# automl/TransformersCanDoBayesianInference

Hardware: AMD Instinct MI355X
Metric: synthetic datasets/sec (GP prior, bptt=2000) (higher is better)
Workload: dtype fp16; 1 GPU; priors.fast_gp, bptt=2000, num_features=18, emsize=512, nhead=4, nhid=1024, nlayers=6, 1000 bars (BASELINE.json configs[1]); per_gpu_batch=64, global_batch=64, aggregate_k_gradients=1, aggregate_streams=0, aggregate_stacked=False, seq_len=2000, parallelism=dp1, micro_batch_streams=2, eval_pos=weighted sampler(2000)

## Files before the change

transformerscandobayesianinference_amd/csrc/gemm_tn.hip:

```cpp
#include <type_traits>
#include "pfn_device.h"
#include "pfn_kernels.h"

namespace pfn {

PFN_DEV int xcd_remap(int bid, int nwg) {
  const int q = nwg >> 3, r = nwg & 7, xcd = bid & 7;
  return (xcd < r ? xcd * (q + 1) : r * (q + 1) + (xcd - r) * q) + (bid >> 3);
}
typedef __attribute__((address_space(1))) const void gvoid_t;
typedef __attribute__((address_space(3))) void lvoid_t;

constexpr int TN_BMK = 32;

template <typename T>
__global__ __launch_bounds__(256, 2) void gemm_tn_kernel(GemmTN g) {
  constexpr int RB = 128 * sizeof(T);
  constexpr int TILE = TN_BMK * RB;
  extern __shared__ __attribute__((aligned(16))) char smem_raw[];
  LdsPtr smem = lds_cast(smem_raw);
  auto tileA = [&](int buf) { return smem + buf * 2 * TILE; };
  auto tileB = [&](int buf) { return smem + buf * 2 * TILE + TILE; };

  const int p0 = blockIdx.y * 128, q0 = blockIdx.x * 128;
  const int colsA = min(128, g.P - p0), colsB = min(128, g.Q - q0);
  const long mbeg = (long)blockIdx.z * g.m_chunk;
  const long mend = min((long)g.M, mbeg + g.m_chunk);
  if (mbeg >= mend) return;
  const T* A = reinterpret_cast<const T*>(g.A) + mbeg * g.lda + p0;
  const T* B = reinterpret_cast<const T*>(g.B) + mbeg * g.ldb + q0;

  const int wave = threadIdx.x >> 6, lane = threadIdx.x & 63;
  const int wp = wave >> 1, wq = wave & 1;

  f32x16 acc[2][2];
#pragma unroll
  for (int i = 0; i < 2; ++i)
#pragma unroll
    for (int j = 0; j < 2; ++j)
#pragma unroll
      for (int r = 0; r < 16; ++r) acc[i][j][r] = 0.f;

  TileStage<T, TN_BMK, RB, 256> sa, sb;
  const int rows_total = (int)(mend - mbeg);
  const int nt = (rows_total + TN_BMK - 1) / TN_BMK;
  const bool do_colsum = g.colsum != nullptr && blockIdx.x == 0;
  constexpr int EPC = 16 / sizeof(T);
  float csum[EPC];
#pragma unroll
  for (int e = 0; e < EPC; ++e) csum[e] = 0.f;
  auto add_colsum = [&]() {
    if (!do_colsum) return;
#pragma unroll
    for (int i = 0; i < sa.PER; ++i) {
      if constexpr (sizeof(T) == 2) {
        const X8<T> v = __builtin_bit_cast(X8<T>, sa.regs[i]);
#pragma unroll
        for (int e = 0; e < 8; ++e) csum[e] += (float)v[e];
      } else {
        const f32x4 v = __builtin_bit_cast(f32x4, sa.regs[i]);
#pragma unroll
        for (int e = 0; e < 4; ++e) csum[e] += v[e];
      }
    }
  };
  sa.issue(A, g.lda, rows_total, colsA);
  sb.issue(B, g.ldb, rows_total, colsB);
  add_colsum();
  sa.template commit<true>(tileA(0));
  sb.template commit<true>(tileB(0));
  __syncthreads();
  for (int t = 0; t < nt; ++t) {
    const int cur = t & 1;
    if (t + 1 < nt) {
      const long r1 = (long)(t + 1) * TN_BMK;
      sa.issue(A + r1 * g.lda, g.lda, rows_total - (int)r1, colsA);
      sb.issue(B + r1 * g.ldb, g.ldb, rows_total - (int)r1, colsB);
      add_colsum();
    }
    const lds_char* ta = tileA(cur);
    const lds_char* tb = tileB(cur);
#pragma unroll
    for (int ks = 0; ks < TN_BMK; ks += 16) {
      Frag<T> fa[2], fb[2];
#pragma unroll
      for (int i = 0; i < 2; ++i) fa[i] = load_frag_tr<T, RB, 1>(ta, ks, wp * 64 + i * 32);
#pragma unroll
      for (int j = 0; j < 2; ++j) fb[j] = load_frag_tr<T, RB, 1>(tb, ks, wq * 64 + j * 32);
#pragma unroll
      for (int i = 0; i < 2; ++i)
#pragma unroll
        for (int j = 0; j < 2; ++j) acc[i][j] = mma32(fa[i], fb[j], acc[i][j]);
    }
    if (t + 1 < nt) {
      sa.template commit<true>(tileA(cur ^ 1));
      sb.template commit<true>(tileB(cur ^ 1));
    }
    __syncthreads();
  }

  const float osc = loss_scale_down(g.scale_amax);
  if (do_colsum) {
    constexpr int NCH = RB / 16;
    float* red = reinterpret_cast<float*>(smem_raw);
#pragma unroll
    for (int e = 0; e < EPC; ++e) red[threadIdx.x * EPC + e] = csum[e];
    __syncthreads();
    if (threadIdx.x < NCH) {
#pragma unroll
      for (int e = 0; e < EPC; ++e) {
        float t = 0.f;
        for (int j = 0; j < 256 / NCH; ++j) t += red[(j * NCH + threadIdx.x) * EPC + e];
        const int col = p0 + threadIdx.x * EPC + e;
        if (col < g.P) unsafeAtomicAdd(g.colsum + col, t * loss_scale_down(g.scale_amax));
      }
    }
  }
#pragma unroll
  for (int i = 0; i < 2; ++i)
#pragma unroll
    for (int j = 0; j < 2; ++j)
#pragma unroll
      for (int r = 0; r < 16; ++r) {
        const int p = p0 + wp * 64 + i * 32 + acc_row(r, lane);
        const int q = q0 + wq * 64 + j * 32 + (lane & 31);
        if (p < g.P && q < g.Q) {
          float* c = g.C + (long)p * g.ldc + q;
          if (g.atomic) unsafeAtomicAdd(c, acc[i][j][r] * osc);
          else *c = acc[i][j][r] * osc;
        }
      }
}

constexpr int TNB_KT = 64;
constexpr int TNB_NS = 2;
constexpr int TNB_TILE = TNB_KT * 512;
constexpr int TNB_LDS = TNB_NS * 2 * TNB_TILE;
static_assert(TNB_LDS <= 160 * 1024, "weight-gradient stages do not fit the CU's LDS");
constexpr long TN_GROUP_MAX_SPLIT_BYTES = 0x7ffffff0L;

template <int NW> struct TnStager {
  static constexpr int NP = TNB_KT / 2 / NW;
  DmaRsrc ra, rb;
  unsigned a_lo, a_hi, b_lo, b_hi;
  unsigned step_a, step_b;
  int va[NP], vb[NP];
  int wave, srow, mask;
  PFN_DEV void init(const TnProblem& pr, long mbeg, int rows, int p0, int q0, int wave_, int lane, int debug_mask) {
    const long lda2 = pr.lda * 2, ldb2 = pr.ldb * 2;
    ra = make_dma_rsrc(reinterpret_cast<const char*>(pr.A) + mbeg * lda2 + p0 * 2, (rows - 1) * lda2 + 512);
    rb = make_dma_rsrc(reinterpret_cast<const char*>(pr.B) + mbeg * ldb2 + q0 * 2, (rows - 1) * ldb2 + 512);
    a_lo = ra.w[0]; a_hi = ra.w[1]; b_lo = rb.w[0]; b_hi = rb.w[1];
    step_a = __builtin_amdgcn_readfirstlane((unsigned)(TNB_KT * lda2));
    step_b = __builtin_amdgcn_readfirstlane((unsigned)(TNB_KT * ldb2));
    wave = wave_; srow = 0; mask = debug_mask;
    const int row0 = wave * 2 + (lane >> 5);
    const int colb = ((((lane & 31) >> 2) ^ (row0 & 3)) * 32 + (lane & 3) * 8) * 2;
#pragma unroll
    for (int i = 0; i < NP; ++i) {
      va[i] = (row0 + 2 * NW * i) * (int)lda2 + colb;
      vb[i] = (row0 + 2 * NW * i) * (int)ldb2 + colb;
    }
  }
  PFN_DEV void issue(LdsPtr slot) {
    LdsPtr ta = slot + wave * 1024;
    LdsPtr tb = ta + TNB_TILE;
#pragma unroll
    for (int i = 0; i < NP; ++i) {
      dma16(ra, ta + i * NW * 1024, va[i]);
      dma16(rb, tb + i * NW * 1024, vb[i]);
    }
    dma_rsrc_advance(ra, step_a);
    dma_rsrc_advance(rb, step_b);
    srow += TNB_KT;
    if ((srow & mask) == 0) { ra.w[0] = a_lo; ra.w[1] = a_hi; rb.w[0] = b_lo; rb.w[1] = b_hi; }
  }
};

template <typename T>
__global__ __launch_bounds__(512, 1) void gemm_tn_big_kernel(GemmTNGroup g) {
  extern __shared__ __attribute__((aligned(16))) char smem_raw[];
  LdsPtr smem = lds_cast(smem_raw);

  const int ntiles = g.tile_start[g.n];
  const int id = xcd_remap(blockIdx.x, ntiles * g.splits);
  const int split = id / ntiles, tile = id % ntiles;
  int pi = 0;
  while (tile >= g.tile_start[pi + 1]) ++pi;
  const TnProblem& pr = g.p[pi];
  const int tq = pr.Q / 256;
  const int tl = tile - g.tile_start[pi];
  const int p0 = (tl / tq) * 256, q0 = (tl % tq) * 256;
  const long mbeg = (long)split * g.m_chunk;
  const long mend = min((long)g.M, mbeg + g.m_chunk);
  const int rows_total = (int)(mend - mbeg);
  if (rows_total <= 0) return;

  const int wave = __builtin_amdgcn_readfirstlane(threadIdx.x >> 6), lane = threadIdx.x & 63;
  const int wp = wave >> 2, wq = wave & 3;

  TnStager<8> stg;
  stg.init(pr, mbeg, rows_total, p0, q0, wave, lane, g.debug_mask);

  f32x16 acc[4][2];
#pragma unroll
  for (int i = 0; i < 4; ++i)
#pragma unroll
    for (int j = 0; j < 2; ++j)
#pragma unroll
      for (int r = 0; r < 16; ++r) acc[i][j][r] = 0.f;
  f32x16 cs;
#pragma unroll
  for (int r = 0; r < 16; ++r) cs[r] = 0.f;
  const bool do_colsum = pr.colsum != nullptr && q0 == 0;
  Frag<T> ones;
#pragma unroll
  for (int e = 0; e < 8; ++e) ones.v[e] = (T)1.0f;

  const int nt = (rows_total + TNB_KT - 1) / TNB_KT;
#pragma unroll
  for (int st = 0; st < TNB_NS - 1; ++st)
    if (st < nt) stg.issue(smem + st * 2 * TNB_TILE);
  auto main_loop = [&nt, &stg, &smem, &wq, &wp, &acc, &cs, &ones](auto with_colsum) {
    constexpr bool CS = decltype(with_colsum)::value;
    int slot = 0, slot_next = 1;
    for (int t = 0; t < nt; ++t) {
      wait_vm_barrier<0>();
      const bool more = t + 1 < nt;
      LdsPtr ta = smem + slot * 2 * TNB_TILE;
      LdsPtr tb = ta + TNB_TILE;
#pragma unroll
      for (int ks = 0; ks < TNB_KT; ks += 16) {
        Frag<T> fa[4], fb[2];
#pragma unroll
        for (int j = 0; j < 2; ++j) fb[j] = load_frag_tr<T, 512, 1>(tb, ks, wq * 64 + j * 32);
#pragma unroll
        for (int i = 0; i < 4; ++i) fa[i] = load_frag_tr<T, 512, 1>(ta, ks, wp * 128 + i * 32);
#pragma unroll
        for (int i = 0; i < 4; ++i)
#pragma unroll
          for (int j = 0; j < 2; ++j) acc[i][j] = mma32(fa[i], fb[j], acc[i][j]);
        if constexpr (CS) cs = mma32(load_frag_tr<T, 512, 1>(ta, ks, wp * 128 + wq * 32), ones, cs);
        if (ks == 0) {
          PFN_PIN_LDS_MFMA();
          if (more) stg.issue(smem + slot_next * 2 * TNB_TILE);
          PFN_PIN_LDS_MFMA();
        }
      }
      slot_next = slot;
      slot = slot + 1 == TNB_NS ? 0 : slot + 1;
    }
  };
  if (do_colsum) main_loop(std::true_type{});
  else main_loop(std::false_type{});

  const int pv = pr.Pv > 0 ? pr.Pv : pr.P;
  const float osc = loss_scale_down(g.scale_amax);
  if (do_colsum && (lane & 31) == 0) {
#pragma unroll
    for (int r = 0; r < 16; ++r) {
      const int pp = p0 + wp * 128 + wq * 32 + acc_row(r, lane);
      if (pp < pv) unsafeAtomicAdd(pr.colsum + pp, cs[r] * osc);
    }
  }
  const bool atomic = true;
#pragma unroll
  for (int i = 0; i < 4; ++i)
#pragma unroll
    for (int j = 0; j < 2; ++j)
#pragma unroll
      for (int r = 0; r < 16; ++r) {
        const int pp = p0 + wp * 128 + i * 32 + acc_row(r, lane);
        const int qq = q0 + wq * 64 + j * 32 + (lane & 31);
        float* c = pr.C + (long)pp * pr.ldc + qq;
        if (pp >= pv) continue;
        if (atomic) unsafeAtomicAdd(c, acc[i][j][r] * osc);
        else *c += acc[i][j][r] * osc;
      }
}

constexpr int TNW_NW = 4;
template <typename T>
__global__ __launch_bounds__(TNW_NW * 64, 1) void gemm_tn_wide_kernel(GemmTNGroup g) {
  extern __shared__ __attribute__((aligned(16))) char smem_raw[];
  LdsPtr smem = lds_cast(smem_raw);
  const int ntiles = g.tile_start[g.n];
  const int id = xcd_remap(blockIdx.x, ntiles * g.splits);
  const int split = id / ntiles, tile = id % ntiles;
  int pi = 0;
  while (tile >= g.tile_start[pi + 1]) ++pi;
  const TnProblem& pr = g.p[pi];
  const int tq = pr.Q / 256;
  const int tl = tile - g.tile_start[pi];
  const int p0 = (tl / tq) * 256, q0 = (tl % tq) * 256;
  const long mbeg = (long)split * g.m_chunk;
  const long mend = min((long)g.M, mbeg + g.m_chunk);
  const int rows_total = (int)(mend - mbeg);
  if (rows_total <= 0) return;
  const int wave = __builtin_amdgcn_readfirstlane(threadIdx.x >> 6), lane = threadIdx.x & 63;
  const int wp = wave >> 1, wq = wave & 1;

  TnStager<TNW_NW> stg;
  stg.init(pr, mbeg, rows_total, p0, q0, wave, lane, g.debug_mask);

  f32x16 acc[4][4];
#pragma unroll
  for (int i = 0; i < 4; ++i)
#pragma unroll
    for (int j = 0; j < 4; ++j)
#pragma unroll
      for (int r = 0; r < 16; ++r) acc[i][j][r] = 0.f;
  float cs[2] = {0.f, 0.f};
  const bool do_colsum = pr.colsum != nullptr && q0 == 0;

  const int nt = (rows_total + TNB_KT - 1) / TNB_KT;
  struct Frs { Frag<T> a[4], b[4]; };
  auto main_loop = [&](auto with_colsum) {
    constexpr bool CS = decltype(with_colsum)::value;
    Frs f0, f1;
    auto ld = [&](Frs& f, const lds_char* ta, const lds_char* tb, int ks) {
#pragma unroll
      for (int j = 0; j < 4; ++j) f.b[j] = load_frag_tr<T, 512, 1>(tb, ks, wq * 128 + j * 32);
#pragma unroll
      for (int i = 0; i < 4; ++i) f.a[i] = load_frag_tr<T, 512, 1>(ta, ks, wp * 128 + i * 32);
    };
    auto mm = [&](const Frs& f) {
#pragma unroll
      for (int i = 0; i < 4; ++i)
#pragma unroll
        for (int j = 0; j < 4; ++j) acc[i][j] = mma32(f.a[i], f.b[j], acc[i][j]);
      if constexpr (CS) {
#pragma unroll
        for (int c = 0; c < 2; ++c)
#pragma unroll
          for (int e = 0; e < 8; ++e) cs[c] += (float)(wq ? f.a[2 + c] : f.a[c]).v[e];
      }
    };
    auto enter_stage = [&](int t, int slot) {
      wait_vm_barrier<0>();
      if (t + 1 < nt) stg.issue(smem + (slot ^ 1) * 2 * TNB_TILE);
    };
    int slot = 0;
    enter_stage(0, slot);
    ld(f0, smem, smem + TNB_TILE, 0);
    for (int t = 0; t < nt; ++t) {
      const lds_char* ta = smem + slot * 2 * TNB_TILE;
      const lds_char* tb = ta + TNB_TILE;
      ld(f1, ta, tb, 16);
      PFN_PIN_LDS_MFMA();
      mm(f0);
      PFN_PIN_LDS_MFMA();
      ld(f0, ta, tb, 32);
      PFN_PIN_LDS_MFMA();
      mm(f1);
      PFN_PIN_LDS_MFMA();
      ld(f1, ta, tb, 48);
      PFN_PIN_LDS_MFMA();
      mm(f0);
      PFN_PIN_LDS_MFMA();
      slot ^= 1;
      if (t + 1 < nt) {
        enter_stage(t + 1, slot);
        const lds_char* tan = smem + slot * 2 * TNB_TILE;
        ld(f0, tan, tan + TNB_TILE, 0);
      }
      PFN_PIN_LDS_MFMA();
      mm(f1);
      PFN_PIN_LDS_MFMA();
    }
  };
  stg.issue(smem);
  if (do_colsum) main_loop(std::true_type{});
  else main_loop(std::false_type{});

  const int pv = pr.Pv > 0 ? pr.Pv : pr.P;
  const float osc = loss_scale_down(g.scale_amax);
  if (do_colsum) {
#pragma unroll
    for (int c = 0; c < 2; ++c) {
      const float s = cs[c] + __shfl_xor(cs[c], 32, 64);
      const int pp = p0 + wp * 128 + (2 * wq + c) * 32 + (lane & 31);
      if (lane < 32 && pp < pv) unsafeAtomicAdd(pr.colsum + pp, s * osc);
    }
  }
#pragma unroll
  for (int i = 0; i < 4; ++i)
#pragma unroll
    for (int j = 0; j < 4; ++j)
#pragma unroll
      for (int r = 0; r < 16; ++r) {
        const int pp = p0 + wp * 128 + i * 32 + acc_row(r, lane);
        const int qq = q0 + wq * 128 + j * 32 + (lane & 31);
        if (pp < pv) unsafeAtomicAdd(pr.C + (long)pp * pr.ldc + qq, acc[i][j][r] * osc);
      }
}

static bool aligned16(const void* p) { return (reinterpret_cast<uintptr_t>(p) & 15) == 0; }

static int g_tn_debug_wrap = 0;
void set_gemm_tn_debug_wrap(int rows) { g_tn_debug_wrap = rows; }
static bool g_tn_wide = false;
void set_gemm_tn_group_waves(int waves) { g_tn_wide = waves == 4; }

int launch_gemm_tn(GemmTN g, int precision, hipStream_t stream) {
  if (g.M <= 0 || g.P <= 0 || g.Q <= 0) return PFN_OK;
  const size_t es = prec_esize(precision);
  if ((g.lda * es) % 16 || (g.ldb * es) % 16 || !aligned16(g.A) || !aligned16(g.B)) return PFN_ERR_ALIGNMENT;
  const int tp = (g.P + 127) / 128, tq = (g.Q + 127) / 128;
  int splits = (1024 + tp * tq - 1) / (tp * tq);
  const int max_splits = (g.M + 4 * TN_BMK - 1) / (4 * TN_BMK);
  if (splits > max_splits) splits = max_splits;
  if (g.max_splits > 0 && splits > g.max_splits) splits = g.max_splits;
  if (splits < 1) splits = 1;
  if (!g.atomic) splits = 1;
  int chunk = (g.M + splits - 1) / splits;
  chunk = (chunk + TN_BMK - 1) / TN_BMK * TN_BMK;
  splits = (g.M + chunk - 1) / chunk;
  g.m_chunk = chunk;
  const size_t lds = 4 * TN_BMK * 128 * es;
  PFN_DISPATCH_OP(precision, hipLaunchKernelGGL(gemm_tn_kernel<T>, dim3(tq, tp, splits), dim3(256), lds, stream, g));
  return hipGetLastError() == hipSuccess ? PFN_OK : PFN_ERR_LAUNCH;
}

bool gemm_tn_group_supported(const TnProblem& p) {
  return p.P % 256 == 0 && p.Q % 256 == 0 && (p.lda * 2) % 16 == 0 && (p.ldb * 2) % 16 == 0 && aligned16(p.A) && aligned16(p.B);
}

int launch_gemm_tn_group(GemmTNGroup g, int precision, hipStream_t stream) {
  if (g.n <= 0 || g.M <= 0) return PFN_OK;
  if (g.n > TN_GROUP_MAX) return PFN_ERR_ARGUMENT;
  if (!prec_is16(precision)) return PFN_ERR_UNSUPPORTED;
  int tiles = 0;
  for (int i = 0; i < g.n; ++i) {
    if (!gemm_tn_group_supported(g.p[i])) return PFN_ERR_UNSUPPORTED;
    g.tile_start[i] = tiles;
    tiles += (g.p[i].P / 256) * (g.p[i].Q / 256);
  }
  g.tile_start[g.n] = tiles;
  int splits = g.splits;
  if (splits <= 0) {
    splits = 8;
    for (int sp = 1; sp <= 8; ++sp) {
      const int blocks = tiles * sp, rounds = (blocks + 255) / 256;
      if (blocks >= 0.9 * rounds * 256) { splits = sp; break; }
    }
  }
  const int max_splits = (g.M + 4 * TNB_KT - 1) / (4 * TNB_KT);
  if (splits > max_splits) splits = max_splits;
  int chunk = (g.M + splits - 1) / splits;
  chunk = (chunk + TNB_KT - 1) / TNB_KT * TNB_KT;
  splits = (g.M + chunk - 1) / chunk;
  g.splits = splits;
  g.m_chunk = chunk;
  for (int i = 0; i < g.n; ++i) {
    const TnProblem& p = g.p[i];
    if (p.lda < 256 || p.ldb < 256 || (long)chunk * p.lda * 2 > TN_GROUP_MAX_SPLIT_BYTES || (long)chunk * p.ldb * 2 > TN_GROUP_MAX_SPLIT_BYTES) return PFN_ERR_UNSUPPORTED;
  }
  const int wrap = g_tn_debug_wrap;
  g.debug_mask = wrap >= TNB_KT && (wrap & (wrap - 1)) == 0 ? wrap - 1 : 0x7fffffff;
  if (g_tn_wide) {
    static LdsAllowance allow_w[2];
    if (precision == PFN_PREC_FP16) {
      allow_w[1].ensure(gemm_tn_wide_kernel<f16>, TNB_LDS);
      hipLaunchKernelGGL(gemm_tn_wide_kernel<f16>, dim3(tiles * splits), dim3(TNW_NW * 64), TNB_LDS, stream, g);
    } else {
      allow_w[0].ensure(gemm_tn_wide_kernel<bf16>, TNB_LDS);
      hipLaunchKernelGGL(gemm_tn_wide_kernel<bf16>, dim3(tiles * splits), dim3(TNW_NW * 64), TNB_LDS, stream, g);
    }
    return hipGetLastError() == hipSuccess ? PFN_OK : PFN_ERR_LAUNCH;
  }
  static LdsAllowance allowance[2];
  if (precision == PFN_PREC_FP16) {
    allowance[1].ensure(gemm_tn_big_kernel<f16>, TNB_LDS);
    hipLaunchKernelGGL(gemm_tn_big_kernel<f16>, dim3(tiles * splits), dim3(512), TNB_LDS, stream, g);
  } else {
    allowance[0].ensure(gemm_tn_big_kernel<bf16>, TNB_LDS);
    hipLaunchKernelGGL(gemm_tn_big_kernel<bf16>, dim3(tiles * splits), dim3(512), TNB_LDS, stream, g);
  }
  return hipGetLastError() == hipSuccess ? PFN_OK : PFN_ERR_LAUNCH;
}

}
```

transformerscandobayesianinference_amd/csrc/pfn_kernels.h:

```cpp
#pragma once
#include "pfn_host.h"

namespace pfn {

#define PFN_DISPATCH_OP(prec, ...)                                                          \
  do {                                                                                      \
    if ((prec) == PFN_PREC_BF16) { using T = ::pfn::bf16_t; __VA_ARGS__; }                  \
    else if ((prec) == PFN_PREC_FP16) { using T = ::pfn::f16_t; __VA_ARGS__; }              \
    else { using T = float; __VA_ARGS__; }                                                  \
  } while (0)
typedef __bf16 bf16_t;
typedef _Float16 f16_t;

__host__ __device__ inline unsigned dropout_site_seed(unsigned long long seed, int layer, int site) {
  return mix32(mix32((unsigned)seed ^ (0x9E3779B1u * (unsigned)(layer * 4 + site + 1))) ^ (unsigned)(seed >> 32));
}
__host__ __device__ inline unsigned dropout_pair_seed(unsigned site_seed, int pair) { return mix32(site_seed ^ (0xC2B2AE35u * (unsigned)(pair + 1))); }
__host__ __device__ inline unsigned dropout_threshold(float p) {
  const double t = (double)p * 4294967296.0;
  return t >= 4294967295.0 ? 0xffffffffu : (unsigned)t;
}
__host__ __device__ inline bool dropout_keep(unsigned s, unsigned i, unsigned j, unsigned thr) {
  return mix32(s ^ (i * 0x9E3779B1u) ^ (j * 0x85EBCA77u)) >= thr;
}

enum : int {
  EPI_BIAS = 1,
  EPI_GELU = 2,
  EPI_GELU_BWD = 4,
  EPI_RESID = 8,
  EPI_OUT_F32 = 16,
  EPI_OUT_T = 32,
  EPI_OUT2_T = 64,
  EPI_ACCUM = 128,
  EPI_RESID_T = 256,
  EPI_ROWDOT = 512,
  EPI_ROWSHIFT = 1024,
};

struct GemmNT {
  const void* A; long lda;
  const void* B; long ldb;
  int M, N, K;
  int flags;
  const float* bias;
  const void* aux; long ld_aux;
  const float* resid; long ld_resid;
  float* out_f32; long ld_out_f32;
  void* out_t; long ld_out_t;
  void* out2_t; long ld_out2;
  int vec_ok;
  int wide_t;
  float* rowdot; const float* rd_lse; long rd_lse2_off; int rd_S, rd_H, rd_D;
  const float* rowshift; long rs_ld; int rs_S, rs_n0, rs_n1;
};
int launch_key_shift(const void* x_t, const void* w_k_t, float* kshift, int B, int S, int E, int sep, const int* sep_of, int precision, hipStream_t s);
int launch_gemm_nt(const GemmNT& g, int precision, hipStream_t stream);
bool gemm_nt_rowdot_fused(const GemmNT& g, int precision);
void set_gemm_nt_big_mode(int mode);
void set_gemm_ln_rows64(int on);

struct GemmTN {
  const void* A; long lda;
  const void* B; long ldb;
  float* C; long ldc;
  int M, P, Q;
  int atomic;
  int m_chunk;
  float* colsum;
  int max_splits;
  const float* scale_amax;
};
int launch_gemm_tn(GemmTN g, int precision, hipStream_t stream);

constexpr int TN_GROUP_MAX = 26;
struct TnProblem {
  const void* A; const void* B; float* C; float* colsum;
  long lda, ldb, ldc;
  int P, Q;
  int Pv;
};
struct GemmTNGroup {
  TnProblem p[TN_GROUP_MAX];
  int tile_start[TN_GROUP_MAX + 1];
  int n, M, splits, m_chunk;
  int debug_mask;
  const float* scale_amax;
};
void set_gemm_tn_debug_wrap(int rows);
void set_gemm_tn_group_waves(int waves);
struct GemmLN {
  const void* A; long lda;
  const void* B; long ldb;
  int M, N, K;
  const float* bias;
  const float* resid;
  const void* ry; const float* rmean; const float* rrstd; const float* rgamma; const float* rbeta;
  const float* gamma; const float* beta; float eps;
  void* y; float* mean; float* rstd; void* x_t;
  float* x_f32;
  int y16;
};
bool gemm_ln_supported(const GemmLN& g);
int launch_gemm_ln(const GemmLN& g, int precision, hipStream_t stream);

struct GemmLNB {
  const void* A; long lda;
  const void* B; long ldb;
  int M, N, K;
  const void* aux;
  const void* y; const float* mean; const float* rstd; const float* gamma;
  void* dx_t;
  float* dgamma; float* dbeta;
  const float* scale_amax;
  int y16;
};
bool gemm_lnbwd_supported(const GemmLNB& g);
int launch_gemm_lnbwd(const GemmLNB& g, int precision, hipStream_t stream);

bool gemm_tn_group_supported(const TnProblem& p);
int launch_gemm_tn_group(GemmTNGroup g, int precision, hipStream_t stream);

struct AttnArgs {
  const void* qkv; void* ctx; float* lse;
  int B, S, E, H, sep;
  const int* sep_of;
  int q_from_sep;
  union {
    struct {
      const void* dctx; void* dqkv; float* delta;
      void* ds;
      int ds_rows, ds_ld;
      int parts;
      int zero_delta;
    };
    struct {
      const void* kv; long kv_ld, kv_sb;
      float* part_o;
      float* part_ml;
      int split_keys;
    };
  };
  int pingpong;
  const void* xq;
  const void* wq;
  const float* bq;
  int q_store;
  int q_begin;
  float p_drop;
  unsigned drop_seed;
};
int attn_cache_splits(int B, int n, int E, int H, int sep, int precision);
int launch_attn_fwd_cache(const AttnArgs& a, int precision, hipStream_t stream);
void set_attn_cache_split_cap(int splits);
struct AttnCacheBwdArgs {
  const void* qkv;
  const void* ctx;
  const float* lse;
  const void* dctx;
  void* dqkv;
  const void* kv; long kv_ld, kv_sb;
  float* part_dq;
  int B, S, E, H, sep;
  int split_keys;
  const int* sep_of;
};
int launch_clamp_sep_of(const int* src, int* dst, int B, int hi, hipStream_t stream);
int launch_attn_bwd_cache(const AttnCacheBwdArgs& a, int precision, hipStream_t stream);
void set_attn_pingpong(int mask);
enum : int { ATTN_BWD_DELTA = 1, ATTN_BWD_KV = 2, ATTN_BWD_DQ = 4 };
int64_t attn_bwd_ds_bytes(int B, int S, int H, int precision);
int launch_attn_fwd(const AttnArgs& a, int precision, hipStream_t stream);
bool attn_fwd_can_fuse_q(int E, int H, int precision);
int launch_attn_bwd(const AttnArgs& a, int precision, hipStream_t stream);

int launch_cast_params(const float* src, void* dst_t, long n, int precision, hipStream_t s);
constexpr int TRANSPOSE_GROUP_MAX = 64;
struct TransposeGroup {
  int n = 0, blocks = 0;
  long src_off[TRANSPOSE_GROUP_MAX], dst_off[TRANSPOSE_GROUP_MAX];
  int rows[TRANSPOSE_GROUP_MAX], cols[TRANSPOSE_GROUP_MAX], ld_dst[TRANSPOSE_GROUP_MAX], first_block[TRANSPOSE_GROUP_MAX];
};
void transpose_group_add(TransposeGroup& g, long src_off, long dst_off, int rows, int cols, int ld_dst);
int launch_transpose_cast_group(const float* src, void* dst, const TransposeGroup& g, int precision, hipStream_t s);
int launch_transpose_cast(const float* src, void* dst_t, int rows, int cols, long ld_dst, int precision, hipStream_t s);
int launch_cast_rows(const float* src, long ld_src, void* dst_t, long ld_dst, long R, int C, int precision, hipStream_t s, const float* scale_amax = nullptr);
int launch_absmax(const float* x, long n, float* amax, hipStream_t s);
int set_loss_scale_target(int log2_target);
int launch_scale_copy(const float* src, float* dst, long n, const float* scale_amax, hipStream_t s);

struct EmbedArgs {
  const float* x; long x_st, x_sb;
  const float* y; long y_st, y_sb;
  const float* wx; const float* bx;
  const float* wy; const float* by;
  float* out_f32; void* out_t;
  void* xaug_t;
  int xaug_ld;
  const float* xaug_amax;
  int S, B, nf, E, sep;
  const int* sep_of;
};
constexpr int EMB_MAX_FEATURES = 1022;
__host__ __device__ inline int emb_aug_width(int nf) { return nf + 2 <= 32 ? 32 : nf + 2 <= 64 ? 64 : nf + 2 <= 128 ? 128 : 0; }
int launch_embed_fwd(const EmbedArgs& a, int precision, hipStream_t s);
int launch_embed_colmax(const EmbedArgs& a, float* amax, hipStream_t s);
__device__ inline int xaug_col_exp(const float* amax, int f) {
  if (!amax) return 0;
  const float m = amax[f];
  if (!(m > 0.f) || !(m <= 3.402823466e38f)) return 0;
  const int e = ilogbf(m);
  return e < -126 ? -126 : e;
}
struct EmbedBwdArgs {
  const float* dsrc; const float* x; long x_st, x_sb; const float* y; long y_st, y_sb;
  float* dwx; float* dbx; float* dwy; float* dby;
  int S, B, nf, E, sep;
  const int* sep_of;
  int single_block;
  const float* scale_amax;
};
int launch_embed_bwd(const EmbedBwdArgs& a, hipStream_t s);
int launch_embed_grad_scatter(const float* acc, float* dwx, float* dwy, float* dby, int E, int nf, const float* xaug_amax, hipStream_t s);
struct EmbedInGradArgs {
  const void* dsrc; int dsrc_prec;
  const float* wx; const float* wy;
  float* dx; long dx_st, dx_sb;
  float* dy; long dy_st, dy_sb;
  int S, B, nf, E, sep;
  const float* scale_amax;
};
int launch_embed_input_grad(const EmbedInGradArgs& a, hipStream_t s);

int launch_sbe_to_bse(const float* src, float* out_f32, void* out_t, int S, int B, int E, int precision, hipStream_t s);
int launch_bse_to_sbe(const float* src_bse, float* dst_sbe, int S, int B, int E, hipStream_t s, const float* scale_amax = nullptr);

int launch_layernorm_fwd(const void* x, const float* gamma, const float* beta, float* y_f32, void* y_t,
                         float* mean, float* rstd, long rows, int E, float eps, int precision, hipStream_t s, int x_is_t = 0);
int launch_layernorm_bwd(const void* dy, int dy_is_t, const void* x, const float* gamma, const float* mean, const float* rstd,
                         float* dx_f32, void* dx_t, float* dgamma, float* dbeta, float* dbias_extra,
                         long rows, int E, int precision, hipStream_t s, float* partials = nullptr, const float* scale_amax = nullptr, int x_is_t = 0);
constexpr int LNB_MAX_BLOCKS = 512;
int launch_colsum(const void* a_t, long lda, long rows, int cols, float* out, int precision, hipStream_t s);

int launch_dropout_add(float* y, const float* resid, long rows, int cols, unsigned site_seed, float p, hipStream_t s);
int launch_dropout_scale(const void* src, void* dst, const void* src2, void* dst2, long rows, int cols, unsigned site_seed, float p, int precision, hipStream_t s);
int launch_gather_test_rows(const float* src_bse, void* dst_t, int S, int B, int E, int sep, int precision, hipStream_t s);
int launch_gather_rows_ragged(const void* src_bs, void* dst, int S, int B, long row_bytes, const int* sep_of, const long* row_off, hipStream_t s);
int launch_scatter_rows_ragged(const void* src, void* dst_bs, int S, int B, long row_bytes, const int* sep_of, const long* row_off, int zero_from_block, hipStream_t s);
int launch_zero_row_prefix_ragged(void* base, int S, int B, const int* sep_of, long row_bytes, long width_bytes, hipStream_t s);
int launch_gather_test_rows_ragged(const float* src_bse, void* dst_t, int S, int B, int E, const int* sep_of, const long* row_off, int precision, hipStream_t s);
int launch_scatter_test_rows_ragged(const float* src, void* dst_bse_t, int S, int B, int E, const int* sep_of, const long* row_off, int precision, hipStream_t s);
int launch_scatter_test_rows(const float* src, void* dst_bse_t, int S, int B, int E, int sep, int precision, hipStream_t s);
int launch_gather_rows(const void* src_bs, void* dst_tb, int S, int B, long row_bytes, int sep, hipStream_t s);
int launch_scatter_rows(const void* src_tb, void* dst_bs, int S, int B, long row_bytes, int sep, int zero_from, hipStream_t s);
int launch_zero_row_prefix(void* base, int S, int B, int nrows, long row_bytes, long width_bytes, hipStream_t s);

}
```

Measured before the change: 2580 datasets/s.

## Add balanced stream-K style scheduler for grouped weight-gradient TN GEMM

Result: no change. 2604 datasets/s, median of 6 (+0.9%).

```diff
diff --git a/transformerscandobayesianinference_amd/csrc/gemm_tn.hip b/transformerscandobayesianinference_amd/csrc/gemm_tn.hip
--- a/transformerscandobayesianinference_amd/csrc/gemm_tn.hip
+++ b/transformerscandobayesianinference_amd/csrc/gemm_tn.hip
@@ -1,3 +1,4 @@
+#include <algorithm>
 #include <type_traits>
 #include "pfn_device.h"
 #include "pfn_kernels.h"
@@ -138,6 +139,7 @@
 constexpr int TNB_LDS = TNB_NS * 2 * TNB_TILE;
 static_assert(TNB_LDS <= 160 * 1024, "weight-gradient stages do not fit the CU's LDS");
 constexpr long TN_GROUP_MAX_SPLIT_BYTES = 0x7ffffff0L;
+constexpr int TN_BAL_MIN_TILES = 32;
 
 template <int NW> struct TnStager {
   static constexpr int NP = TNB_KT / 2 / NW;
@@ -178,21 +180,13 @@
 };
 
 template <typename T>
-__global__ __launch_bounds__(512, 1) void gemm_tn_big_kernel(GemmTNGroup g) {
-  extern __shared__ __attribute__((aligned(16))) char smem_raw[];
-  LdsPtr smem = lds_cast(smem_raw);
-
-  const int ntiles = g.tile_start[g.n];
-  const int id = xcd_remap(blockIdx.x, ntiles * g.splits);
-  const int split = id / ntiles, tile = id % ntiles;
+PFN_DEV void tn_big_tile(const GemmTNGroup& g, LdsPtr smem, int tile, long mbeg, long mend) {
   int pi = 0;
   while (tile >= g.tile_start[pi + 1]) ++pi;
   const TnProblem& pr = g.p[pi];
   const int tq = pr.Q / 256;
   const int tl = tile - g.tile_start[pi];
   const int p0 = (tl / tq) * 256, q0 = (tl % tq) * 256;
-  const long mbeg = (long)split * g.m_chunk;
-  const long mend = min((long)g.M, mbeg + g.m_chunk);
   const int rows_total = (int)(mend - mbeg);
   if (rows_total <= 0) return;
 
@@ -254,6 +248,9 @@
   if (do_colsum) main_loop(std::true_type{});
   else main_loop(std::false_type{});
 
+#ifdef PFN_TNB_NO_FLUSH
+  if (g.M > 0) return;
+#endif
   const int pv = pr.Pv > 0 ? pr.Pv : pr.P;
   const float osc = loss_scale_down(g.scale_amax);
   if (do_colsum && (lane & 31) == 0) {
@@ -277,6 +274,28 @@
         if (atomic) unsafeAtomicAdd(c, acc[i][j][r] * osc);
         else *c += acc[i][j][r] * osc;
       }
+}
+
+template <typename T>
+__global__ __launch_bounds__(512, 1) void gemm_tn_big_kernel(GemmTNGroup g) {
+  extern __shared__ __attribute__((aligned(16))) char smem_raw[];
+  const int ntiles = g.tile_start[g.n];
+  const int id = xcd_remap(blockIdx.x, ntiles * g.splits);
+  const int split = id / ntiles, tile = id % ntiles;
+  const long mbeg = (long)split * g.m_chunk;
+  tn_big_tile<T>(g, lds_cast(smem_raw), tile, mbeg, min((long)g.M, mbeg + g.m_chunk));
+}
+
+template <typename T>
+__global__ __launch_bounds__(512, 1) void gemm_tn_balanced_kernel(GemmTNGroup g) {
+  extern __shared__ __attribute__((aligned(16))) char smem_raw[];
+  for (int seg = 0; seg < g.bal.segments; ++seg) {
+    const TnSegment sg = tn_balanced_segment(g.bal, blockIdx.x, seg);
+    if (sg.count == 0) continue;
+    __syncthreads();
+    const long mbeg = (long)sg.first * TNB_KT;
+    tn_big_tile<T>(g, lds_cast(smem_raw), sg.tile, mbeg, min((long)g.M, mbeg + (long)sg.count * TNB_KT));
+  }
 }
 
 constexpr int TNW_NW = 4;
@@ -426,6 +445,40 @@
   return p.P % 256 == 0 && p.Q % 256 == 0 && (p.lda * 2) % 16 == 0 && (p.ldb * 2) % 16 == 0 && aligned16(p.A) && aligned16(p.B);
 }
 
+static int device_cus() {
+  static std::atomic<int> cus[16];
+  int dev = 0;
+  (void)hipGetDevice(&dev);
+  int n = cus[dev & 15].load(std::memory_order_relaxed);
+  if (n == 0) {
+    if (hipDeviceGetAttribute(&n, hipDeviceAttributeMultiprocessorCount, dev) != hipSuccess) n = -1;
+    cus[dev & 15].store(n, std::memory_order_relaxed);
+  }
+  return n;
+}
+
+static int launch_gemm_tn_balanced(GemmTNGroup g, int tiles, int precision, hipStream_t stream) {
+  const int cus = device_cus();
+  if (g_tn_wide || cus < 8 || cus % 8) return PFN_ERR_UNSUPPORTED;
+  g.bal = tn_balanced_make(tiles, g.M, cus);
+  if (g.bal.segments > TN_BAL_MAX_SEGMENTS) return PFN_ERR_UNSUPPORTED;
+  const long seg_rows = (long)std::min(g.bal.nt, g.bal.L / 8 + 1) * TNB_KT;
+  for (int i = 0; i < g.n; ++i) {
+    const TnProblem& p = g.p[i];
+    if (p.lda < 256 || p.ldb < 256 || seg_rows * p.lda * 2 > TN_GROUP_MAX_SPLIT_BYTES || seg_rows * p.ldb * 2 > TN_GROUP_MAX_SPLIT_BYTES) return PFN_ERR_UNSUPPORTED;
+  }
+  g.splits = 1; g.m_chunk = g.M;
+  static LdsAllowance allowance[2];
+  if (precision == PFN_PREC_FP16) {
+    allowance[1].ensure(gemm_tn_balanced_kernel<f16>, TNB_LDS);
+    hipLaunchKernelGGL(gemm_tn_balanced_kernel<f16>, dim3(8 * g.bal.C), dim3(512), TNB_LDS, stream, g);
+  } else {
+    allowance[0].ensure(gemm_tn_balanced_kernel<bf16>, TNB_LDS);
+    hipLaunchKernelGGL(gemm_tn_balanced_kernel<bf16>, dim3(8 * g.bal.C), dim3(512), TNB_LDS, stream, g);
+  }
+  return hipGetLastError() == hipSuccess ? PFN_OK : PFN_ERR_LAUNCH;
+}
+
 int launch_gemm_tn_group(GemmTNGroup g, int precision, hipStream_t stream) {
   if (g.n <= 0 || g.M <= 0) return PFN_OK;
   if (g.n > TN_GROUP_MAX) return PFN_ERR_ARGUMENT;
@@ -437,12 +490,20 @@
     tiles += (g.p[i].P / 256) * (g.p[i].Q / 256);
   }
   g.tile_start[g.n] = tiles;
+  const int wrap = g_tn_debug_wrap;
+  g.debug_mask = wrap >= TNB_KT && (wrap & (wrap - 1)) == 0 ? wrap - 1 : 0x7fffffff;
+  if (g.splits == -1) return launch_gemm_tn_balanced(g, tiles, precision, stream);
   int splits = g.splits;
   if (splits <= 0) {
     splits = 8;
+    bool whole_rounds = false;
     for (int sp = 1; sp <= 8; ++sp) {
       const int blocks = tiles * sp, rounds = (blocks + 255) / 256;
-      if (blocks >= 0.9 * rounds * 256) { splits = sp; break; }
+      if (blocks >= 0.9 * rounds * 256) { splits = sp; whole_rounds = blocks == rounds * 256; break; }
+    }
+    if (tiles >= TN_BAL_MIN_TILES && !whole_rounds && !g_tn_wide) {
+      const int rc = launch_gemm_tn_balanced(g, tiles, precision, stream);
+      if (rc != PFN_ERR_UNSUPPORTED) return rc;
     }
   }
   const int max_splits = (g.M + 4 * TNB_KT - 1) / (4 * TNB_KT);
@@ -456,8 +517,6 @@
     const TnProblem& p = g.p[i];
     if (p.lda < 256 || p.ldb < 256 || (long)chunk * p.lda * 2 > TN_GROUP_MAX_SPLIT_BYTES || (long)chunk * p.ldb * 2 > TN_GROUP_MAX_SPLIT_BYTES) return PFN_ERR_UNSUPPORTED;
   }
-  const int wrap = g_tn_debug_wrap;
-  g.debug_mask = wrap >= TNB_KT && (wrap & (wrap - 1)) == 0 ? wrap - 1 : 0x7fffffff;
   if (g_tn_wide) {
     static LdsAllowance allow_w[2];
     if (precision == PFN_PREC_FP16) {
diff --git a/transformerscandobayesianinference_amd/csrc/pfn_kernels.h b/transformerscandobayesianinference_amd/csrc/pfn_kernels.h
--- a/transformerscandobayesianinference_amd/csrc/pfn_kernels.h
+++ b/transformerscandobayesianinference_amd/csrc/pfn_kernels.h
@@ -1,5 +1,6 @@
 #pragma once
 #include "pfn_host.h"
+#include "tn_schedule.h"
 
 namespace pfn {
 
@@ -86,6 +87,7 @@
   int n, M, splits, m_chunk;
   int debug_mask;
   const float* scale_amax;
+  TnBalanced bal;
 };
 void set_gemm_tn_debug_wrap(int rows);
 void set_gemm_tn_group_waves(int waves);
diff --git a/transformerscandobayesianinference_amd/csrc/tn_schedule.h b/transformerscandobayesianinference_amd/csrc/tn_schedule.h
--- /dev/null
+++ b/transformerscandobayesianinference_amd/csrc/tn_schedule.h
@@ -0,0 +1,66 @@
+#pragma once
+
+#if defined(__HIPCC__)
+#define PFN_SCHED_FN __host__ __device__ inline
+#else
+#define PFN_SCHED_FN inline
+#endif
+
+namespace pfn {
+
+constexpr int TN_BAL_STAGE = 64;
+constexpr int TN_BAL_MAX_SEGMENTS = 8;
+
+struct TnBalanced {
+  int C;
+  int nt;
+  int cols_full;
+  int r, f, ns;
+  int L;
+  int segments;
+};
+
+struct TnSegment { int tile, first, count; };
+
+PFN_SCHED_FN TnBalanced tn_balanced_make(int tiles, int M, int cus) {
+  TnBalanced s;
+  s.C = cus / 8;
+  s.nt = (M + TN_BAL_STAGE - 1) / TN_BAL_STAGE;
+  s.cols_full = tiles / s.C;
+  s.r = tiles % s.C;
+  s.f = s.r ? s.C / s.r : 0;
+  s.ns = s.r ? (s.nt + s.f - 1) / s.f : 0;
+  s.L = s.cols_full * s.nt + s.ns;
+  const int cols = s.cols_full + (s.r ? 1 : 0);
+  const int bound = (cols + 7) / 8 + 1;
+  s.segments = bound < cols ? bound : cols;
+  return s;
+}
+
+PFN_SCHED_FN int tn_balanced_lo(const TnBalanced& s, int x) { return (int)((long)x * s.L / 8); }
+
+PFN_SCHED_FN TnSegment tn_balanced_segment(const TnBalanced& s, int bid, int seg) {
+  TnSegment out = {0, 0, 0};
+  const int x = bid & 7, c = bid >> 3;
+  const int lo = tn_balanced_lo(s, x), hi = tn_balanced_lo(s, x + 1);
+  const int full_len = s.cols_full * s.nt;
+  const int k = (lo < full_len ? lo / s.nt : s.cols_full) + seg;
+  if (c >= s.C || k > s.cols_full) return out;
+  const int cb = k * s.nt;
+  const int ce = k < s.cols_full ? cb + s.nt : s.L;
+  const int a = (lo > cb ? lo : cb) - cb, b = (hi < ce ? hi : ce) - cb;
+  if (b <= a) return out;
+  if (k < s.cols_full) {
+    out.tile = k * s.C + c; out.first = a; out.count = b - a;
+    return out;
+  }
+  if (c >= s.r * s.f) return out;
+  const int j = c / s.r;
+  const int base = (int)((long)j * s.nt / s.f), len = (int)((long)(j + 1) * s.nt / s.f) - base;
+  const int e = b < len ? b : len;
+  if (e <= a) return out;
+  out.tile = s.cols_full * s.C + c % s.r; out.first = base + a; out.count = e - a;
+  return out;
+}
+
+}
```
